# SHI-Labs/SH-GAN

Measured on AMD Instinct MI355X. Metric: generator images/sec, higher is better.
Workload: dtype f32

## Files before the change

### sh-gan_amd/csrc/conv_wino_poly.hip

```cpp
#include "wino_common.h"
#include <stdlib.h>
#include <type_traits>

__device__ __attribute__((aligned(16))) float shg_poly_zeros[64];

struct PolySub {
    const float* wu;
    int nby, nbx;
    int tiles_x, tiles_y;
    int n_ttiles;
};
struct PolyParams {
    const float* x;
    float* y;
    const float* in_scale;
    int NB, I, O, OP, H, W;
    int n_otiles, nchunk;
    PolySub a, b;
    const float* wt;
    int IPK, n_strip_tiles;
    int PH2, PP;
    const float* bias;
    const float* residual;
    int act;
    float alpha, gain, clamp;
    int cps;
    long part_stride;
};

namespace poly {
constexpr int KC = 8, BO = 64, BT = 64;
constexpr int V_SZ = 16 * KC * BT;
constexpr int NT = 1024;
constexpr int NXF = KC;

enum { UA = 0, UB = 1, DA = 2, DB = 3 };

template <int SCHEME, int TY, int TX, int NBX>
struct Geo {
    static constexpr bool A = SCHEME == UA || SCHEME == DA;
    static_assert(NBX > 0 || TY * TX == BT, "64 blocks per tile");
    static_assert(NBX == 0 || A, "flat tiling is for the 3x3 blocks of schemes UA / DA");
    static constexpr int BS = A ? 3 : 2;
    static constexpr int RMAX = NBX ? (NBX - 1 + BT + NBX - 1) / NBX : TY;
    static constexpr int PH = A ? 3 * RMAX + 1 : 2 * TY + 1;
    static constexpr int PW = SCHEME == UA ? ((3 * (NBX ? NBX : TX) + 1 + 3 + 3) / 4) * 4
                            : SCHEME == DA ? (NBX ? ((3 * NBX + 1 + 3) / 4) * 4 : ((3 * TX + 1 + 3 + 3) / 4) * 4)
                            : 2 * TX + 4;
    static constexpr int DB_W0 = 2 * TX, DB_W1 = 2 * TX + 4, DB_W2 = 2 * TX;
    static constexpr int DB_N0 = (2 * TY + 1) * DB_W0, DB_N1 = 2 * TY * DB_W1, DB_N2 = 2 * TY * DB_W2;
    static constexpr int RP = SCHEME == DB ? DB_N0 + DB_N1 + DB_N2 : PH * PW;
    static constexpr int PW4 = PW / 4, PATCH4 = RP / 4, R_SZ = KC * RP;
    static constexpr int NPIECE = (PATCH4 + 63) / 64;
};
}

template <int SCHEME, int TY, int TX, int NBX>
__device__ __forceinline__ void poly_body(const PolyParams& p, const PolySub& q, const int bid, float* __restrict__ Vl,
                                          float* __restrict__ Rl) {
    using namespace poly;
    using G = Geo<SCHEME, TY, TX, NBX>;
    constexpr int PW = G::PW, PW4 = G::PW4, PATCH4 = G::PATCH4, RP = G::RP, R_SZ = G::R_SZ, BS = G::BS, NPIECE = G::NPIECE;
    constexpr bool FLAT = NBX > 0;
    constexpr bool DOWN = SCHEME == DA || SCHEME == DB;
    const int c0 = DOWN ? 0 : blockIdx.y * p.cps, nch = DOWN ? p.nchunk : min(p.cps, p.nchunk - c0), iend = min(p.I, (c0 + nch) * poly::KC);

    const int tid = threadIdx.x;
    const int lane = tid & 63, wave = __builtin_amdgcn_readfirstlane(tid >> 6);
    const int l31 = lane & 31, half = lane >> 5;

    const int nwork = q.n_ttiles * p.n_otiles;
    const int work = shg_xcd_remap(bid, nwork);
    const int otile = work / q.n_ttiles;
    const int ttile = work - otile * q.n_ttiles;
    const int txb = ttile % q.tiles_x;
    const int tyb = (ttile / q.tiles_x) % q.tiles_y;
    const int n = ttile / (q.tiles_x * q.tiles_y);
    const int id0 = txb * BT;
    const int by0 = FLAT ? id0 / (NBX ? NBX : 1) : tyb * TY, bx0 = FLAT ? 0 : txb * TX;
    const int o0 = otile * BO;
    const int HW = DOWN ? p.PH2 * p.PP : p.H * p.W;
    const int wy0 = DOWN ? BS * by0 : BS * by0 - 1;
    const int wx0 = SCHEME == UA ? ((3 * bx0 - 1) & ~3) : SCHEME == DA ? ((3 * bx0) & ~3) : SCHEME == UB ? 2 * bx0 - 4 : 2 * bx0;
    const int coff = (DOWN ? BS * bx0 : BS * bx0 - 1) - wx0;

    const bool xformer = wave < NXF;
    constexpr int NLD = 16 - NXF;
    constexpr int CPL = (KC + NLD - 1) / NLD;
    int roff[NPIECE];
#pragma unroll
    for (int j = 0; j < NPIECE; ++j) {
        const int e = j * 64 + lane;
        if constexpr (SCHEME == DB) {
            constexpr int N0 = G::DB_N0 / 4, N1 = G::DB_N1 / 4, W0 = G::DB_W0 / 4, W1 = G::DB_W1 / 4, W2 = G::DB_W2 / 4;
            const int pl = e < N0 ? 1 : (e < N0 + N1 ? 2 : 3);
            const int r4 = e < N0 ? e : (e < N0 + N1 ? e - N0 : e - N0 - N1);
            const int w4 = pl == 1 ? W0 : (pl == 2 ? W1 : W2);
            const int py = r4 / w4, p4 = r4 - py * w4;
            const int iy = wy0 + py, ix = wx0 + 4 * p4;
            const bool ok = e < PATCH4 && iy < p.PH2 && ix + 3 < p.PP;
            roff[j] = ok ? (pl * p.NB + n) * p.I * HW + iy * p.PP + ix : -1;
        } else {
            const int py = e / PW4, p4 = e - py * PW4;
            const int iy = wy0 + py, ix = wx0 + 4 * p4;
            if constexpr (SCHEME == DA) {
                const bool ok = e < PATCH4 && iy < p.PH2 && ix + 3 < p.PP;
                roff[j] = ok ? n * p.I * HW + iy * p.PP + ix : -1;
            } else {
                const bool ok = e < PATCH4 && iy >= 0 && iy < p.H && ix >= 0 && ix + 3 < p.W;
                roff[j] = ok ? n * p.I * HW + iy * p.W + ix : -1;
            }
        }
    }
    const bool ract_last = lane < PATCH4 - 64 * (NPIECE - 1);
    auto dma_raw = [&](int c, int buf) __attribute__((always_inline)) {
#pragma unroll
        for (int q = 0; q < CPL; ++q) {
            const int k = (wave - NXF) * CPL + q;
            if (k >= KC) continue;
            const int ch = (c0 + c) * KC + k;
            const bool chok = ch < iend;
#pragma unroll
            for (int j = 0; j < NPIECE; ++j) {
                const float* src = (chok && roff[j] >= 0) ? p.x + ((long)roff[j] + (long)ch * HW) : shg_poly_zeros;
                if (j < NPIECE - 1 || ract_last)
                    __builtin_amdgcn_global_load_lds((const __attribute__((address_space(1))) void*)src,
                                                     (__attribute__((address_space(3))) void*)(Rl + buf * R_SZ + k * RP + j * 256), 16, 0, 0);
            }
        }
    };

    constexpr int NU = KC / 4;
    const size_t ustride = (size_t)16 * 64 * KC / 4;
    const f32x4* ubase = reinterpret_cast<const f32x4*>(q.wu + (((size_t)otile * p.nchunk * 16 + wave) * 64 + lane) * KC) + (size_t)c0 * ustride;
    f32x4 ua[NU], ub[NU];
    auto load_u = [&](f32x4 (&dst)[NU], int c) __attribute__((always_inline)) {
#pragma unroll
        for (int j = 0; j < NU; ++j) dst[j] = ubase[(size_t)c * ustride + j];
    };

    const int tty = FLAT ? (id0 + lane) / (NBX ? NBX : 1) - by0 : lane / TX;
    const int ttx = FLAT ? (id0 + lane) % (NBX ? NBX : 1) : lane % TX;
    const float* rbase = Rl + wave * RP + (SCHEME == DB ? 0 : (BS * tty) * PW + BS * ttx + coff);
    float* vbase = Vl + wave * BT + lane;
    float scv[2];
#pragma unroll
    for (int v = 0; v < 2; ++v) {
        const int ch = (v * 64 + lane) * KC + wave;
        scv[v] = (p.in_scale && xformer && ch < p.I) ? p.in_scale[(long)n * p.I + ch] : 1.f;
    }
    auto transform = [&](int c, int buf) __attribute__((always_inline)) {
        const int ca = c0 + c;
        const float sc = __builtin_bit_cast(float, __builtin_amdgcn_readlane(__builtin_bit_cast(int, ca < 64 ? scv[0] : scv[1]), ca & 63));
        const float* rb = rbase + buf * R_SZ;
        float* vb = vbase + buf * V_SZ;
        if constexpr (SCHEME == DB) {
            const float* we = rb + (2 * tty) * G::DB_W0 + 2 * ttx;
#pragma unroll
            for (int cc = 0; cc < 2; ++cc) {
                const float d0 = we[cc] * sc, d1 = we[G::DB_W0 + cc] * sc, d2 = we[2 * G::DB_W0 + cc] * sc;
                vb[(0 * 2 + cc) * KC * BT] = d0 - d1;
                vb[(1 * 2 + cc) * KC * BT] = d1;
                vb[(2 * 2 + cc) * KC * BT] = d2 - d1;
            }
            const float* wo = rb + G::DB_N0 + (2 * tty) * G::DB_W1 + 2 * ttx;
#pragma unroll
            for (int r = 0; r < 2; ++r) {
                const float e0 = wo[r * G::DB_W1] * sc, e1 = wo[r * G::DB_W1 + 1] * sc, e2 = wo[r * G::DB_W1 + 2] * sc;
                vb[(6 + r * 3 + 0) * KC * BT] = e0 - e1;
                vb[(6 + r * 3 + 1) * KC * BT] = e1;
                vb[(6 + r * 3 + 2) * KC * BT] = e2 - e1;
            }
            const float* wq = rb + G::DB_N0 + G::DB_N1 + (2 * tty) * G::DB_W2 + 2 * ttx;
#pragma unroll
            for (int r = 0; r < 2; ++r)
#pragma unroll
                for (int cc = 0; cc < 2; ++cc) vb[(12 + r * 2 + cc) * KC * BT] = wq[r * G::DB_W2 + cc] * sc;
        } else if constexpr (G::A) {
            float f[4][4];
#pragma unroll
            for (int r = 0; r < 4; ++r) {
                const float d0 = rb[r * PW] * sc, d1 = rb[r * PW + 1] * sc, d2 = rb[r * PW + 2] * sc, d3 = rb[r * PW + 3] * sc;
                f[r][0] = d0 - d2; f[r][1] = d1 + d2; f[r][2] = d2 - d1; f[r][3] = d1 - d3;
                if (r == 1) __builtin_amdgcn_sched_barrier(0);
            }
#pragma unroll
            for (int j = 0; j < 4; ++j) {
                vb[(0 * 4 + j) * KC * BT] = f[0][j] - f[2][j];
                vb[(1 * 4 + j) * KC * BT] = f[1][j] + f[2][j];
                vb[(2 * 4 + j) * KC * BT] = f[2][j] - f[1][j];
                vb[(3 * 4 + j) * KC * BT] = f[1][j] - f[3][j];
            }
        } else {
            float d[3][3];
#pragma unroll
            for (int r = 0; r < 3; ++r)
#pragma unroll
                for (int cc = 0; cc < 3; ++cc) d[r][cc] = rb[r * PW + cc] * sc;
#pragma unroll
            for (int cc = 1; cc < 3; ++cc) {
                vb[(0 * 2 + cc - 1) * KC * BT] = d[0][cc] - d[1][cc];
                vb[(1 * 2 + cc - 1) * KC * BT] = d[1][cc];
                vb[(2 * 2 + cc - 1) * KC * BT] = d[2][cc] - d[1][cc];
            }
#pragma unroll
            for (int r = 1; r < 3; ++r) {
                vb[(6 + (r - 1) * 3 + 0) * KC * BT] = d[r][0] - d[r][1];
                vb[(6 + (r - 1) * 3 + 1) * KC * BT] = d[r][1];
                vb[(6 + (r - 1) * 3 + 2) * KC * BT] = d[r][2] - d[r][1];
            }
#pragma unroll
            for (int r = 1; r < 3; ++r)
#pragma unroll
                for (int cc = 1; cc < 3; ++cc) vb[(12 + (r - 1) * 2 + cc - 1) * KC * BT] = d[r][cc];
        }
    };

    f32x16 acc[2][2];
#pragma unroll
    for (int ob = 0; ob < 2; ++ob)
#pragma unroll
        for (int tb = 0; tb < 2; ++tb)
#pragma unroll
            for (int r = 0; r < 16; ++r) acc[ob][tb][r] = 0.f;
    const float* bbase = Vl + (wave * KC + half) * BT + l31;

    load_u(ua, 0);
    if (!xformer) {
        dma_raw(0, 0);
        if (nch > 1) dma_raw(1, 1);
    }
    asm volatile("s_waitcnt vmcnt(0)" ::: "memory");
    __syncthreads();
    if (xformer) transform(0, 0);
    __syncthreads();

    float b[2][2], apend[2];
    auto mma = [&](float a0, float a1, int buf) __attribute__((always_inline)) {
#pragma unroll
        for (int tb = 0; tb < 2; ++tb) acc[0][tb] = __builtin_amdgcn_mfma_f32_32x32x2f32(a0, b[buf][tb], acc[0][tb], 0, 0, 0);
#pragma unroll
        for (int tb = 0; tb < 2; ++tb) acc[1][tb] = __builtin_amdgcn_mfma_f32_32x32x2f32(a1, b[buf][tb], acc[1][tb], 0, 0, 0);
    };
    auto chunk = [&](auto par, int c) __attribute__((always_inline)) {
        constexpr int PAR = decltype(par)::value;
        f32x4 (&ucur)[NU] = PAR ? ub : ua;
        f32x4 (&unxt)[NU] = PAR ? ua : ub;
        const bool more = c + 1 < nch;
        const float* bb = bbase + PAR * V_SZ;
        auto fetch = [&](int ks, int buf) __attribute__((always_inline)) {
#pragma unroll
            for (int tb = 0; tb < 2; ++tb) b[buf][tb] = bb[(ks * 2) * BT + tb * 32];
        };
        fetch(0, 0);
        __builtin_amdgcn_sched_barrier(0);
        if (c > 0) mma(apend[0], apend[1], 1);
        __builtin_amdgcn_sched_barrier(0);
        if (more) load_u(unxt, c + 1);
        if (!xformer) {
            if (c + 2 < nch) dma_raw(c + 2, PAR);
        } else if (more) {
            transform(c + 1, PAR ^ 1);
        }
        __builtin_amdgcn_sched_barrier(0);
#pragma unroll
        for (int ks = 0; ks < KC / 2 - 1; ++ks) {
            fetch(ks + 1, (ks + 1) & 1);
            __builtin_amdgcn_sched_barrier(0);
            mma(ucur[(ks * 2) / 4][(ks * 2) % 4], ucur[(ks * 2 + 1) / 4][(ks * 2 + 1) % 4], ks & 1);
        }
        apend[0] = ucur[(KC - 2) / 4][(KC - 2) % 4];
        apend[1] = ucur[(KC - 1) / 4][(KC - 1) % 4];
        asm volatile("s_waitcnt lgkmcnt(0)" ::: "memory");
        __syncthreads();
    };
    for (int c = 0; c < nch; c += 2) {
        chunk(std::integral_constant<int, 0>{}, c);
        if (c + 1 < nch) chunk(std::integral_constant<int, 1>{}, c + 1);
    }
    mma(apend[0], apend[1], 1);

    float* Mx = Vl;
    const int PWg = DOWN ? p.W : p.W + 1;
    const long plane = DOWN ? (long)p.H * p.W : (long)(p.H + 1) * PWg;
    const int o_l = tid >> 5, t_l = tid & 31;
    f32x2 pre_part[SCHEME == DB ? 4 : 1][2], pre_res[SCHEME == DB ? 4 : 1][2];
    float pre_bias[2] = {0.f, 0.f};
    if constexpr (SCHEME == DB) {
#pragma unroll
        for (int pass = 0; pass < 4; ++pass) {
            const int ob = pass >> 1, t = (pass & 1) * 32 + t_l;
            const int by = by0 + t / TX, bx = bx0 + t % TX;
            const int o = min(o0 + ob * 32 + o_l, p.O - 1);
            if ((pass & 1) == 0) pre_bias[ob] = p.bias ? p.bias[o] : 0.f;
#pragma unroll
            for (int j = 0; j < 2; ++j) {
                pre_part[pass][j] = f32x2{0.f, 0.f};
                pre_res[pass][j] = f32x2{0.f, 0.f};
                if (by < q.nby && bx < q.nbx && 2 * by + j < p.H) {
                    const long off = ((long)n * p.O + o) * plane + (long)(2 * by + j) * PWg + 2 * bx;
                    pre_part[pass][j] = *reinterpret_cast<const f32x2*>(p.y + off);
                    if (p.residual) pre_res[pass][j] = *reinterpret_cast<const f32x2*>(p.residual + off);
                }
            }
        }
    }
#pragma unroll
    for (int pass = 0; pass < 4; ++pass) {
        const int ob = pass >> 1, tb = pass & 1;
#pragma unroll
        for (int r = 0; r < 16; ++r) {
            const int row = (r & 3) + 8 * (r >> 2) + 4 * half;
            Mx[(wave * 32 + row) * 32 + l31] = acc[ob][tb][r];
        }
        __syncthreads();
        float m[16];
#pragma unroll
        for (int xi = 0; xi < 16; ++xi) m[xi] = Mx[(xi * 32 + o_l) * 32 + t_l];
        const int t = tb * 32 + t_l;
        const int by = FLAT ? (id0 + t) / (NBX ? NBX : 1) : by0 + t / TX, bx = FLAT ? (id0 + t) % (NBX ? NBX : 1) : bx0 + t % TX;
        const int o = o0 + ob * 32 + o_l;
        if (o < p.O && by < q.nby && bx < q.nbx) {
            float* yb = p.y + (DOWN ? 0 : blockIdx.y * p.part_stride) + ((long)n * p.O + o) * plane;
            const long pstride = (long)p.NB * p.O * plane;
            if constexpr (G::A) {
                float t3[3][4];
#pragma unroll
                for (int cc = 0; cc < 4; ++cc) {
                    t3[0][cc] = m[0 * 4 + cc] + m[1 * 4 + cc] + m[2 * 4 + cc];
                    t3[1][cc] = m[1 * 4 + cc] - m[2 * 4 + cc];
                    t3[2][cc] = m[1 * 4 + cc] + m[2 * 4 + cc] - m[3 * 4 + cc];
                }
                constexpr int EXT = DOWN ? 0 : 1;
#pragma unroll
                for (int i = 0; i < 3; ++i) {
                    const int u = 3 * by + i;
                    if (u >= p.H + EXT) continue;
                    const float y0 = t3[i][0] + t3[i][1] + t3[i][2], y1 = t3[i][1] - t3[i][2], y2 = t3[i][1] + t3[i][2] - t3[i][3];
                    float* yr = yb + (long)u * PWg + 3 * bx;
                    yr[0] = y0;
                    if (3 * bx + 1 < p.W + EXT) yr[1] = y1;
                    if (3 * bx + 2 < p.W + EXT) yr[2] = y2;
                }
            } else if constexpr (SCHEME == DB) {
                const int p0 = 2 * by, q0 = 2 * bx;
                const float bs = pre_bias[ob];
#pragma unroll
                for (int j = 0; j < 2; ++j) {
                    if (p0 + j >= p.H) continue;
                    float* yr = yb + (long)(p0 + j) * PWg + q0;
                    const f32x2 part = pre_part[pass][j];
                    const f32x2 rs = pre_res[pass][j];
                    f32x2 out;
#pragma unroll
                    for (int cc = 0; cc < 2; ++cc) {
                        float v = part[cc] + m[j * 2 + cc] + m[(j + 1) * 2 + cc]
                                + m[6 + j * 3 + cc] + m[6 + j * 3 + cc + 1]
                                + m[12 + j * 2 + cc] + bs;
                        v = p.act ? shg_lrelu_agc(v, p.alpha, p.gain, p.clamp) : v * p.gain;
                        out[cc] = v + rs[cc];
                    }
                    *reinterpret_cast<f32x2*>(yr) = out;
                }
            } else {
                const int u0 = 2 * by, v0 = 2 * bx;
                float* yeo = yb + pstride + (long)u0 * PWg + v0;
                float* yoe = yb + 2 * pstride + (long)u0 * PWg + v0;
                float* yoo = yb + 3 * pstride + (long)u0 * PWg + v0;
#pragma unroll
                for (int cc = 0; cc < 2; ++cc) {
                    yeo[cc] = m[0 * 2 + cc] + m[1 * 2 + cc];
                    yeo[PWg + cc] = m[1 * 2 + cc] + m[2 * 2 + cc];
                }
#pragma unroll
                for (int r = 0; r < 2; ++r) {
                    yoe[r * PWg] = m[6 + r * 3] + m[6 + r * 3 + 1];
                    yoe[r * PWg + 1] = m[6 + r * 3 + 1] + m[6 + r * 3 + 2];
                    yoo[r * PWg] = m[12 + r * 2];
                    yoo[r * PWg + 1] = m[12 + r * 2 + 1];
                }
            }
        }
        if (pass < 3) __syncthreads();
    }
}

__device__ __forceinline__ void poly_strip_body(const PolyParams& p, const int tile, const int wave, float* __restrict__ redbuf) {
    float (*red)[16][64] = reinterpret_cast<float (*)[16][64]>(redbuf);
    const float* wt = p.wt;
    const int IPK = p.IPK;
    const int lane = threadIdx.x & 63;
    const int l31 = lane & 31, half = lane >> 5;
    const int nseg_r = (p.W + 31) / 32, nseg_c = (p.H + 31) / 32;
    const int no32 = p.OP / 32;
    const bool live = tile < p.n_strip_tiles;
    int seg = tile % (nseg_r + nseg_c);
    const int ot32 = (tile / (nseg_r + nseg_c)) % no32;
    const int n = live ? tile / ((nseg_r + nseg_c) * no32) : 0;
    const bool col = seg >= nseg_r;
    if (col) seg -= nseg_r;
    const int len = col ? p.H : p.W;
    const int pos = seg * 32 + l31;
    const int tap = col ? 1 * 3 + 2 : 2 * 3 + 1;
    const int HW = p.H * p.W;
    const bool pok = live && pos < len;
    const float* xb = p.x + (long)n * p.I * HW + (pok ? (col ? pos * p.W + p.W - 1 : (p.H - 1) * p.W + pos) : 0);
    const float* wb = wt + ((long)(ot32 >> 1) * IPK + tap) * 64 + (ot32 & 1) * 32 + l31;
    const float* sb = p.in_scale ? p.in_scale + (long)n * p.I : nullptr;
    const int i_lo = blockIdx.y * p.cps * poly::KC, i_hi = min(p.I, i_lo + p.cps * poly::KC);
    const int kper = ((i_hi - i_lo + 7) / 8) * 2;
    const int kbeg = i_lo + wave * kper, kend = min(i_hi, kbeg + kper);
    f32x16 acc;
#pragma unroll
    for (int r = 0; r < 16; ++r) acc[r] = 0.f;
    for (int i0 = kbeg; i0 < kend; i0 += 32) {
        float a[16], bv[16];
#pragma unroll
        for (int k = 0; k < 16; ++k) {
            const int ic = i0 + 2 * k + half;
            const int i = min(ic, p.I - 1);
            a[k] = wb[(long)i * 9 * 64];
            bv[k] = xb[(long)i * HW];
            if (sb) bv[k] *= sb[i];
            if (ic >= kend) a[k] = 0.f;
            if (ic >= kend || !pok) bv[k] = 0.f;
        }
#pragma unroll
        for (int k = 0; k < 16; ++k) acc = __builtin_amdgcn_mfma_f32_32x32x2f32(a[k], bv[k], acc, 0, 0, 0);
    }
#pragma unroll
    for (int r = 0; r < 16; ++r) red[wave][r][lane] = acc[r];
    __syncthreads();
    if (!pok) return;
    const int PWg = p.W + 1;
    const long plane = (long)(p.H + 1) * PWg;
    const long pix = col ? (long)pos * PWg + p.W : (long)p.H * PWg + pos;
    float* yb = p.y + blockIdx.y * p.part_stride + (long)(col ? 2 : 1) * p.NB * p.O * plane + (long)n * p.O * plane + pix;
#pragma unroll
    for (int rr = 0; rr < 4; ++rr) {
        const int r = wave * 4 + rr;
        const float v = red[0][r][lane] + red[1][r][lane] + red[2][r][lane] + red[3][r][lane];
        const int o = ot32 * 32 + (r & 3) + 8 * (r >> 2) + 4 * half;
        if (o < p.O) yb[(long)o * plane] = v;
    }
}

template <int ATY, int ATX, int ANBX, int BTY, int BTX>
__global__ __launch_bounds__(1024) void conv_poly_up_kernel(const PolyParams p) {
    using namespace poly;
    using GA = Geo<UA, ATY, ATX, ANBX>;
    using GB = Geo<UB, BTY, BTX, 0>;
    constexpr int R_MAX = GA::R_SZ > GB::R_SZ ? GA::R_SZ : GB::R_SZ;
    __shared__ __attribute__((aligned(16))) float Vl[2 * V_SZ];
    __shared__ __attribute__((aligned(16))) float Rl[2 * R_MAX];
    const int nA = p.a.n_ttiles * p.n_otiles, nB = p.b.n_ttiles * p.n_otiles;
    if ((int)blockIdx.x < nA) poly_body<UA, ATY, ATX, ANBX>(p, p.a, blockIdx.x, Vl, Rl);
    else if ((int)blockIdx.x < nA + nB) poly_body<UB, BTY, BTX, 0>(p, p.b, blockIdx.x - nA, Vl, Rl);
    else {
        const int wave = threadIdx.x >> 6;
        poly_strip_body(p, (blockIdx.x - nA - nB) * 4 + (wave >> 2), wave & 3, Vl + (wave >> 2) * 4 * 16 * 64);
    }
}

template <int SCHEME, int TY, int TX, int NBX>
__global__ __launch_bounds__(1024) void conv_poly_down_kernel(const PolyParams p) {
    using namespace poly;
    using G = Geo<SCHEME, TY, TX, NBX>;
    __shared__ __attribute__((aligned(16))) float Vl[2 * V_SZ];
    __shared__ __attribute__((aligned(16))) float Rl[2 * G::R_SZ];
    poly_body<SCHEME, TY, TX, NBX>(p, SCHEME == DA ? p.a : p.b, blockIdx.x, Vl, Rl);
}

__global__ __launch_bounds__(256) void poly_weight_kernel(const float* w, const float* scale, float* wu, int O, int I, int OP,
                                                          int nchunk, int flip, int scheme) {
    constexpr int KC = poly::KC;
    const long e = (long)blockIdx.x * 256 + threadIdx.x;
    const long total = (long)OP * nchunk * KC;
    if (e >= total) return;
    const int o = (int)(e % OP);
    const int i = (int)(e / OP);
    float g[3][3];
#pragma unroll
    for (int t = 0; t < 9; ++t) {
        const int tt = flip ? 8 - t : t;
        g[t / 3][t % 3] = (o < O && i < I) ? w[((long)o * I + i) * 9 + tt] * scale[o] : 0.f;
    }
    float u[16];
    if (scheme == poly::UA) {
        const float q00 = g[2][2], q01 = g[2][0], q10 = g[0][2], q11 = g[0][0];
        float gq[4][2];
        gq[0][0] = q00; gq[0][1] = q01;
        gq[1][0] = 0.5f * (q00 + q10); gq[1][1] = 0.5f * (q01 + q11);
        gq[2][0] = 0.5f * (q00 - q10); gq[2][1] = 0.5f * (q01 - q11);
        gq[3][0] = q10; gq[3][1] = q11;
#pragma unroll
        for (int r = 0; r < 4; ++r) {
            u[r * 4 + 0] = gq[r][0];
            u[r * 4 + 1] = 0.5f * (gq[r][0] + gq[r][1]);
            u[r * 4 + 2] = 0.5f * (gq[r][0] - gq[r][1]);
            u[r * 4 + 3] = gq[r][1];
        }
    } else if (scheme == poly::UB) {
        const float g0 = g[0][1], g1 = g[2][1];
        const float h0 = g[1][0], h1 = g[1][2];
#pragma unroll
        for (int cc = 0; cc < 2; ++cc) { u[0 * 2 + cc] = g1; u[1 * 2 + cc] = g0 + g1; u[2 * 2 + cc] = g0; }
#pragma unroll
        for (int r = 0; r < 2; ++r) { u[6 + r * 3 + 0] = h1; u[6 + r * 3 + 1] = h0 + h1; u[6 + r * 3 + 2] = h0; }
#pragma unroll
        for (int k = 0; k < 4; ++k) u[12 + k] = g[1][1];
    } else if (scheme == poly::DA) {
        const float q00 = g[0][0], q01 = g[0][2], q10 = g[2][0], q11 = g[2][2];
        float gq[4][2];
        gq[0][0] = q00; gq[0][1] = q01;
        gq[1][0] = 0.5f * (q00 + q10); gq[1][1] = 0.5f * (q01 + q11);
        gq[2][0] = 0.5f * (q00 - q10); gq[2][1] = 0.5f * (q01 - q11);
        gq[3][0] = q10; gq[3][1] = q11;
#pragma unroll
        for (int r = 0; r < 4; ++r) {
            u[r * 4 + 0] = gq[r][0];
            u[r * 4 + 1] = 0.5f * (gq[r][0] + gq[r][1]);
            u[r * 4 + 2] = 0.5f * (gq[r][0] - gq[r][1]);
            u[r * 4 + 3] = gq[r][1];
        }
    } else {
        const float g0 = g[0][1], g1 = g[2][1];
        const float h0 = g[1][0], h1 = g[1][2];
#pragma unroll
        for (int cc = 0; cc < 2; ++cc) { u[0 * 2 + cc] = g0; u[1 * 2 + cc] = g0 + g1; u[2 * 2 + cc] = g1; }
#pragma unroll
        for (int r = 0; r < 2; ++r) { u[6 + r * 3 + 0] = h0; u[6 + r * 3 + 1] = h0 + h1; u[6 + r * 3 + 2] = h1; }
#pragma unroll
        for (int k = 0; k < 4; ++k) u[12 + k] = g[1][1];
    }
    const int k = i % KC, chunk = i / KC;
    const int ln = (k & 1) * 32 + (o & 31), slot = (k >> 1) * 2 + ((o & 63) >> 5);
    float* dst = wu + ((((long)(o >> 6) * nchunk + chunk) * 16) * 64 + ln) * KC + slot;
#pragma unroll
    for (int xi = 0; xi < 16; ++xi) dst[(long)xi * 64 * KC] = u[xi];
}

extern "C" int shg_conv_weight_prep_up_poly_f32(const float* w, const float* wscale, float* wu_a, float* wu_b, int O, int I, int OP,
                                                int flip, void* stream) {
    SHG_CHECK_ARG(w && wscale && wu_a && wu_b, "weight_prep_up_poly: null pointer");
    SHG_CHECK_ARG(O >= 1 && I >= 1 && OP % 64 == 0 && OP >= O, "weight_prep_up_poly: bad shape");
    const int nchunk = shg_cdiv(I, poly::KC);
    const long total = (long)OP * nchunk * poly::KC;
    hipLaunchKernelGGL(poly_weight_kernel, dim3(shg_cdiv(total, 256)), dim3(256), 0, (hipStream_t)stream, w, wscale, wu_a, O, I, OP,
                       nchunk, flip, (int)poly::UA);
    SHG_CHECK_LAUNCH();
    hipLaunchKernelGGL(poly_weight_kernel, dim3(shg_cdiv(total, 256)), dim3(256), 0, (hipStream_t)stream, w, wscale, wu_b, O, I, OP,
                       nchunk, flip, (int)poly::UB);
    SHG_CHECK_LAUNCH();
    return SHG_OK;
}

extern "C" int shg_conv2d_up_poly_supported(int NB, int I, int O, int H, int W) {
    return (H >= 16 && W >= 16 && H % 2 == 0 && W % 4 == 0 && I <= 128 * poly::KC && NB >= 1 && O >= 1) ? 1 : 0;
}

static int up_poly_plan(PolyParams& p, int NB, int I, int OP, int H, int W) {
    p.n_otiles = OP / 64; p.nchunk = shg_cdiv(I, poly::KC);
    const bool bwide = W >= 32;
    p.b.nby = H / 2; p.b.nbx = W / 2;
    p.b.tiles_x = shg_cdiv(p.b.nbx, bwide ? 16 : 8); p.b.tiles_y = shg_cdiv(p.b.nby, bwide ? 4 : 8);
    p.b.n_ttiles = p.b.tiles_x * p.b.tiles_y * NB;
    p.a.nby = shg_cdiv(H + 1, 3); p.a.nbx = shg_cdiv(W + 1, 3);
    const bool flat = bwide && (p.a.nbx == 11 || p.a.nbx == 22 || p.a.nbx == 43);
    const long w88 = (long)shg_cdiv(p.a.nbx, 8) * shg_cdiv(p.a.nby, 8), w416 = (long)shg_cdiv(p.a.nbx, 16) * shg_cdiv(p.a.nby, 4);
    const bool wide = bwide && w416 < w88;
    if (flat) { p.a.tiles_x = shg_cdiv(p.a.nby * p.a.nbx, 64); p.a.tiles_y = 1; }
    else { p.a.tiles_x = shg_cdiv(p.a.nbx, wide ? 16 : 8); p.a.tiles_y = shg_cdiv(p.a.nby, wide ? 4 : 8); }
    p.a.n_ttiles = p.a.tiles_x * p.a.tiles_y * NB;
    p.IPK = (I + 31) / 32 * 32 * 9;
    p.n_strip_tiles = (shg_cdiv(W, 32) + shg_cdiv(H, 32)) * (OP / 32) * NB;
    if (!bwide) return 0;
    if (flat) return p.a.nbx == 11 ? 1 : (p.a.nbx == 22 ? 2 : 3);
    return wide ? 4 : 5;
}

extern "C" size_t shg_conv2d_up_poly_workspace_bytes(int NB, int I, int O, int OP, int H, int W) {
    if (!shg_conv2d_up_poly_supported(NB, I, O, H, W) || OP < 64) return 0;
    PolyParams p{};
    up_poly_plan(p, NB, I, OP, H, W);
    return shg_wino_split_bytes((long)(p.a.n_ttiles + p.b.n_ttiles) * p.n_otiles, p.nchunk, (size_t)4 * NB * O * (H + 1) * (W + 1) * sizeof(float));
}

extern "C" int shg_conv2d_up_poly_ws_f32(const float* x, const float* wt, const float* wu_a, const float* wu_b, float* y, int NB, int I,
                                         int O, int OP, int H, int W, const float* in_scale, void* workspace, size_t ws_bytes, void* stream) {
    SHG_CHECK_ARG(x && wt && wu_a && wu_b && y, "conv2d_up_poly: null pointer");
    SHG_CHECK_ARG(shg_conv2d_up_poly_supported(NB, I, O, H, W), "conv2d_up_poly: unsupported geometry (use shg_conv2d_f32 mode 2)");
    SHG_CHECK_ARG(OP % 64 == 0 && OP >= O, "conv2d_up_poly: OP must be a multiple of 64 and >= O");
    SHG_CHECK_ARG((long)NB * I * H * W < 2147483647L && 4L * NB * O * (H + 1) * (W + 1) < 2147483647L, "conv2d_up_poly: tensor too large");
    SHG_CHECK_ARG((reinterpret_cast<uintptr_t>(x) & 15) == 0, "conv2d_up_poly: x must be 16-byte aligned");
    hipStream_t s = (hipStream_t)stream;
    PolyParams p{};
    p.x = x; p.y = y; p.in_scale = in_scale;
    p.NB = NB; p.I = I; p.O = O; p.OP = OP; p.H = H; p.W = W;
    p.a.wu = wu_a; p.b.wu = wu_b; p.wt = wt;
    const int variant = up_poly_plan(p, NB, I, OP, H, W);
    const int ks = shg_wino_split((long)(p.a.n_ttiles + p.b.n_ttiles) * p.n_otiles, p.nchunk, (size_t)4 * NB * O * (H + 1) * (W + 1) * sizeof(float),
                                  workspace, ws_bytes, shg_addr(workspace) | shg_addr(y), &p.y, &p.cps, &p.part_stride);
    const dim3 grid((p.a.n_ttiles + p.b.n_ttiles) * p.n_otiles + shg_cdiv(p.n_strip_tiles, 4), ks);
    if (variant == 0) hipLaunchKernelGGL((conv_poly_up_kernel<8, 8, 0, 8, 8>), grid, dim3(poly::NT), 0, s, p);
    else if (variant == 1) hipLaunchKernelGGL((conv_poly_up_kernel<1, 64, 11, 4, 16>), grid, dim3(poly::NT), 0, s, p);
    else if (variant == 2) hipLaunchKernelGGL((conv_poly_up_kernel<1, 64, 22, 4, 16>), grid, dim3(poly::NT), 0, s, p);
    else if (variant == 3) hipLaunchKernelGGL((conv_poly_up_kernel<1, 64, 43, 4, 16>), grid, dim3(poly::NT), 0, s, p);
    else if (variant == 4) hipLaunchKernelGGL((conv_poly_up_kernel<4, 16, 0, 4, 16>), grid, dim3(poly::NT), 0, s, p);
    else hipLaunchKernelGGL((conv_poly_up_kernel<8, 8, 0, 4, 16>), grid, dim3(poly::NT), 0, s, p);
    SHG_CHECK_LAUNCH();
    if (ks > 1) {
        shg_launch_wino_split_reduce((const float*)workspace, y, ks, 4 * NB, O, H + 1, W + 1, nullptr, nullptr, nullptr, 0, 0.f, 0, 0.f, 1.f, -1.f, nullptr, s);
        SHG_CHECK_LAUNCH();
    }
    return SHG_OK;
}

extern "C" int shg_conv2d_up_poly_f32(const float* x, const float* wt, const float* wu_a, const float* wu_b, float* y, int NB, int I,
                                      int O, int OP, int H, int W, const float* in_scale, void* stream) {
    return shg_conv2d_up_poly_ws_f32(x, wt, wu_a, wu_b, y, NB, I, O, OP, H, W, in_scale, nullptr, 0, stream);
}


extern "C" int shg_conv_weight_prep_down_poly_f32(const float* w, const float* wscale, float* wu_a, float* wu_b, int O, int I, int OP,
                                                  int flip, void* stream) {
    SHG_CHECK_ARG(w && wscale && wu_a && wu_b, "weight_prep_down_poly: null pointer");
    SHG_CHECK_ARG(O >= 1 && I >= 1 && OP % 64 == 0 && OP >= O, "weight_prep_down_poly: bad shape");
    const int nchunk = shg_cdiv(I, poly::KC);
    const long total = (long)OP * nchunk * poly::KC;
    hipLaunchKernelGGL(poly_weight_kernel, dim3(shg_cdiv(total, 256)), dim3(256), 0, (hipStream_t)stream, w, wscale, wu_a, O, I, OP,
                       nchunk, flip, (int)poly::DA);
    SHG_CHECK_LAUNCH();
    hipLaunchKernelGGL(poly_weight_kernel, dim3(shg_cdiv(total, 256)), dim3(256), 0, (hipStream_t)stream, w, wscale, wu_b, O, I, OP,
                       nchunk, flip, (int)poly::DB);
    SHG_CHECK_LAUNCH();
    return SHG_OK;
}

extern "C" int shg_conv2d_down_poly_supported(int NB, int I, int O, int OH, int OW) {
    return (OH >= 16 && OW >= 16 && OW % 4 == 0 && OH % 2 == 0 && I <= 128 * poly::KC && NB >= 1 && O >= 1) ? 1 : 0;
}

extern "C" int shg_conv2d_down_poly_f32(const float* xp, const float* wu_a, const float* wu_b, float* y, int NB, int I, int O, int OP,
                                        int OH, int OW, int PP, const float* in_scale, const float* bias, int act, float alpha,
                                        float gain, float clamp, const float* residual, void* stream) {
    SHG_CHECK_ARG(xp && wu_a && wu_b && y, "conv2d_down_poly: null pointer");
    SHG_CHECK_ARG(shg_conv2d_down_poly_supported(NB, I, O, OH, OW), "conv2d_down_poly: unsupported geometry (use shg_conv2d_f32 mode 1)");
    SHG_CHECK_ARG(OP % 64 == 0 && OP >= O, "conv2d_down_poly: OP must be a multiple of 64 and >= O");
    SHG_CHECK_ARG(PP % 4 == 0 && PP >= OW + 1, "conv2d_down_poly: plane pitch must be a multiple of 4 and >= OW + 1");
    SHG_CHECK_ARG(4L * NB * I * (OH + 1) * PP < 2147483647L && (long)NB * O * OH * OW < 2147483647L, "conv2d_down_poly: tensor too large");
    SHG_CHECK_ARG(((reinterpret_cast<uintptr_t>(xp) & 15) | (reinterpret_cast<uintptr_t>(y) & 7) | (reinterpret_cast<uintptr_t>(residual) & 7)) == 0,
                  "conv2d_down_poly: xp must be 16-byte, y / residual 8-byte aligned");
    hipStream_t s = (hipStream_t)stream;
    PolyParams p{};
    p.x = xp; p.y = y; p.in_scale = in_scale; p.bias = bias; p.residual = residual;
    p.NB = NB; p.I = I; p.O = O; p.OP = OP; p.H = OH; p.W = OW; p.PH2 = OH + 1; p.PP = PP;
    p.act = act; p.alpha = alpha; p.gain = gain; p.clamp = clamp;
    p.n_otiles = OP / 64; p.nchunk = shg_cdiv(I, poly::KC);
    p.cps = p.nchunk; p.part_stride = 0;
    p.a.wu = wu_a; p.a.nby = shg_cdiv(OH, 3); p.a.nbx = shg_cdiv(OW, 3);
    const bool flat = p.a.nbx == 11 || p.a.nbx == 22 || p.a.nbx == 43;
    const long w88 = (long)shg_cdiv(p.a.nbx, 8) * shg_cdiv(p.a.nby, 8), w416 = (long)shg_cdiv(p.a.nbx, 16) * shg_cdiv(p.a.nby, 4);
    const bool wide = OW >= 32 && w416 < w88;
    if (flat) { p.a.tiles_x = shg_cdiv(p.a.nby * p.a.nbx, 64); p.a.tiles_y = 1; }
    else { p.a.tiles_x = shg_cdiv(p.a.nbx, wide ? 16 : 8); p.a.tiles_y = shg_cdiv(p.a.nby, wide ? 4 : 8); }
    p.a.n_ttiles = p.a.tiles_x * p.a.tiles_y * NB;
    const dim3 ga(p.a.n_ttiles * p.n_otiles);
    if (flat && p.a.nbx == 11) hipLaunchKernelGGL((conv_poly_down_kernel<poly::DA, 1, 64, 11>), ga, dim3(poly::NT), 0, s, p);
    else if (flat && p.a.nbx == 22) hipLaunchKernelGGL((conv_poly_down_kernel<poly::DA, 1, 64, 22>), ga, dim3(poly::NT), 0, s, p);
    else if (flat) hipLaunchKernelGGL((conv_poly_down_kernel<poly::DA, 1, 64, 43>), ga, dim3(poly::NT), 0, s, p);
    else if (wide) hipLaunchKernelGGL((conv_poly_down_kernel<poly::DA, 4, 16, 0>), ga, dim3(poly::NT), 0, s, p);
    else hipLaunchKernelGGL((conv_poly_down_kernel<poly::DA, 8, 8, 0>), ga, dim3(poly::NT), 0, s, p);
    SHG_CHECK_LAUNCH();
    const bool bwide = OW >= 32, bxwide = OW >= 64;
    p.b.wu = wu_b; p.b.nby = OH / 2; p.b.nbx = OW / 2;
    p.b.tiles_x = shg_cdiv(p.b.nbx, bxwide ? 32 : (bwide ? 16 : 8)); p.b.tiles_y = shg_cdiv(p.b.nby, bxwide ? 2 : (bwide ? 4 : 8));
    p.b.n_ttiles = p.b.tiles_x * p.b.tiles_y * NB;
    const dim3 gb(p.b.n_ttiles * p.n_otiles);
    if (bxwide) hipLaunchKernelGGL((conv_poly_down_kernel<poly::DB, 2, 32, 0>), gb, dim3(poly::NT), 0, s, p);
    else if (bwide) hipLaunchKernelGGL((conv_poly_down_kernel<poly::DB, 4, 16, 0>), gb, dim3(poly::NT), 0, s, p);
    else hipLaunchKernelGGL((conv_poly_down_kernel<poly::DB, 8, 8, 0>), gb, dim3(poly::NT), 0, s, p);
    SHG_CHECK_LAUNCH();
    return SHG_OK;
}
```

Measured before the change: 824.5.

## Specialize winograd main loop on transformer role and tighten LDS DMA issue

Splits the chunk loop into two compile-time variants, one for waves that transform and one for waves that issue raw-input DMA, so the runtime branch leaves the hot loop. Replaces the global_load_lds builtin with inline asm that sets M0 from a scalar (readfirstlane) LDS address. Transform outputs now go to registers first and are stored to LDS together at the end. An explicit vmcnt wait is added before the end-of-chunk barrier. The goal is less branching and better instruction scheduling, at the cost of code size and the fragility of hand-written inline asm and waitcnt encodings.

```diff
diff --git a/sh-gan_amd/csrc/conv_wino_poly.hip b/sh-gan_amd/csrc/conv_wino_poly.hip
--- a/sh-gan_amd/csrc/conv_wino_poly.hip
+++ b/sh-gan_amd/csrc/conv_wino_poly.hip
@@ -123,9 +123,10 @@
 #pragma unroll
             for (int j = 0; j < NPIECE; ++j) {
                 const float* src = (chok && roff[j] >= 0) ? p.x + ((long)roff[j] + (long)ch * HW) : shg_poly_zeros;
+                const unsigned lds = __builtin_amdgcn_readfirstlane(
+                    (unsigned)(size_t)(__attribute__((address_space(3))) void*)(Rl + buf * R_SZ + k * RP + j * 256));
                 if (j < NPIECE - 1 || ract_last)
-                    __builtin_amdgcn_global_load_lds((const __attribute__((address_space(1))) void*)src,
-                                                     (__attribute__((address_space(3))) void*)(Rl + buf * R_SZ + k * RP + j * 256), 16, 0, 0);
+                    asm volatile("s_mov_b32 m0, %0\n\ts_nop 0\n\tglobal_load_lds_dwordx4 %1, off" ::"s"(lds), "v"(src) : "m0", "memory");
             }
         }
     };
@@ -150,32 +151,32 @@
         scv[v] = (p.in_scale && xformer && ch < p.I) ? p.in_scale[(long)n * p.I + ch] : 1.f;
     }
     auto transform = [&](int c, int buf) __attribute__((always_inline)) {
+        float tv[16];
         const int ca = c0 + c;
         const float sc = __builtin_bit_cast(float, __builtin_amdgcn_readlane(__builtin_bit_cast(int, ca < 64 ? scv[0] : scv[1]), ca & 63));
         const float* rb = rbase + buf * R_SZ;
-        float* vb = vbase + buf * V_SZ;
         if constexpr (SCHEME == DB) {
             const float* we = rb + (2 * tty) * G::DB_W0 + 2 * ttx;
 #pragma unroll
             for (int cc = 0; cc < 2; ++cc) {
                 const float d0 = we[cc] * sc, d1 = we[G::DB_W0 + cc] * sc, d2 = we[2 * G::DB_W0 + cc] * sc;
-                vb[(0 * 2 + cc) * KC * BT] = d0 - d1;
-                vb[(1 * 2 + cc) * KC * BT] = d1;
-                vb[(2 * 2 + cc) * KC * BT] = d2 - d1;
+                tv[0 * 2 + cc] = d0 - d1;
+                tv[1 * 2 + cc] = d1;
+                tv[2 * 2 + cc] = d2 - d1;
             }
             const float* wo = rb + G::DB_N0 + (2 * tty) * G::DB_W1 + 2 * ttx;
 #pragma unroll
             for (int r = 0; r < 2; ++r) {
                 const float e0 = wo[r * G::DB_W1] * sc, e1 = wo[r * G::DB_W1 + 1] * sc, e2 = wo[r * G::DB_W1 + 2] * sc;
-                vb[(6 + r * 3 + 0) * KC * BT] = e0 - e1;
-                vb[(6 + r * 3 + 1) * KC * BT] = e1;
-                vb[(6 + r * 3 + 2) * KC * BT] = e2 - e1;
+                tv[6 + r * 3 + 0] = e0 - e1;
+                tv[6 + r * 3 + 1] = e1;
+                tv[6 + r * 3 + 2] = e2 - e1;
             }
             const float* wq = rb + G::DB_N0 + G::DB_N1 + (2 * tty) * G::DB_W2 + 2 * ttx;
 #pragma unroll
             for (int r = 0; r < 2; ++r)
 #pragma unroll
-                for (int cc = 0; cc < 2; ++cc) vb[(12 + r * 2 + cc) * KC * BT] = wq[r * G::DB_W2 + cc] * sc;
+                for (int cc = 0; cc < 2; ++cc) tv[12 + r * 2 + cc] = wq[r * G::DB_W2 + cc] * sc;
         } else if constexpr (G::A) {
             float f[4][4];
 #pragma unroll
@@ -186,10 +187,10 @@
             }
 #pragma unroll
             for (int j = 0; j < 4; ++j) {
-                vb[(0 * 4 + j) * KC * BT] = f[0][j] - f[2][j];
-                vb[(1 * 4 + j) * KC * BT] = f[1][j] + f[2][j];
-                vb[(2 * 4 + j) * KC * BT] = f[2][j] - f[1][j];
-                vb[(3 * 4 + j) * KC * BT] = f[1][j] - f[3][j];
+                tv[0 * 4 + j] = f[0][j] - f[2][j];
+                tv[1 * 4 + j] = f[1][j] + f[2][j];
+                tv[2 * 4 + j] = f[2][j] - f[1][j];
+                tv[3 * 4 + j] = f[1][j] - f[3][j];
             }
         } else {
             float d[3][3];
@@ -199,21 +200,24 @@
                 for (int cc = 0; cc < 3; ++cc) d[r][cc] = rb[r * PW + cc] * sc;
 #pragma unroll
             for (int cc = 1; cc < 3; ++cc) {
-                vb[(0 * 2 + cc - 1) * KC * BT] = d[0][cc] - d[1][cc];
-                vb[(1 * 2 + cc - 1) * KC * BT] = d[1][cc];
-                vb[(2 * 2 + cc - 1) * KC * BT] = d[2][cc] - d[1][cc];
+                tv[0 * 2 + cc - 1] = d[0][cc] - d[1][cc];
+                tv[1 * 2 + cc - 1] = d[1][cc];
+                tv[2 * 2 + cc - 1] = d[2][cc] - d[1][cc];
             }
 #pragma unroll
             for (int r = 1; r < 3; ++r) {
-                vb[(6 + (r - 1) * 3 + 0) * KC * BT] = d[r][0] - d[r][1];
-                vb[(6 + (r - 1) * 3 + 1) * KC * BT] = d[r][1];
-                vb[(6 + (r - 1) * 3 + 2) * KC * BT] = d[r][2] - d[r][1];
+                tv[6 + (r - 1) * 3 + 0] = d[r][0] - d[r][1];
+                tv[6 + (r - 1) * 3 + 1] = d[r][1];
+                tv[6 + (r - 1) * 3 + 2] = d[r][2] - d[r][1];
             }
 #pragma unroll
             for (int r = 1; r < 3; ++r)
 #pragma unroll
-                for (int cc = 1; cc < 3; ++cc) vb[(12 + (r - 1) * 2 + cc - 1) * KC * BT] = d[r][cc];
-        }
+                for (int cc = 1; cc < 3; ++cc) tv[12 + (r - 1) * 2 + cc - 1] = d[r][cc];
+        }
+        float* vb = vbase + buf * V_SZ;
+#pragma unroll
+        for (int xi = 0; xi < 16; ++xi) vb[xi * KC * BT] = tv[xi];
     };
 
     f32x16 acc[2][2];
@@ -242,8 +246,9 @@
 #pragma unroll
         for (int tb = 0; tb < 2; ++tb) acc[1][tb] = __builtin_amdgcn_mfma_f32_32x32x2f32(a1, b[buf][tb], acc[1][tb], 0, 0, 0);
     };
-    auto chunk = [&](auto par, int c) __attribute__((always_inline)) {
+    auto chunk = [&](auto par, auto xf_c, int c) __attribute__((always_inline)) {
         constexpr int PAR = decltype(par)::value;
+        constexpr bool XF = decltype(xf_c)::value;
         f32x4 (&ucur)[NU] = PAR ? ub : ua;
         f32x4 (&unxt)[NU] = PAR ? ua : ub;
         const bool more = c + 1 < nch;
@@ -257,7 +262,7 @@
         if (c > 0) mma(apend[0], apend[1], 1);
         __builtin_amdgcn_sched_barrier(0);
         if (more) load_u(unxt, c + 1);
-        if (!xformer) {
+        if constexpr (!XF) {
             if (c + 2 < nch) dma_raw(c + 2, PAR);
         } else if (more) {
             transform(c + 1, PAR ^ 1);
@@ -271,13 +276,18 @@
         }
         apend[0] = ucur[(KC - 2) / 4][(KC - 2) % 4];
         apend[1] = ucur[(KC - 1) / 4][(KC - 1) % 4];
+        __builtin_amdgcn_s_waitcnt(0x0F70);
         asm volatile("s_waitcnt lgkmcnt(0)" ::: "memory");
         __syncthreads();
     };
-    for (int c = 0; c < nch; c += 2) {
-        chunk(std::integral_constant<int, 0>{}, c);
-        if (c + 1 < nch) chunk(std::integral_constant<int, 1>{}, c + 1);
-    }
+    auto run = [&](auto xf_c) __attribute__((always_inline)) {
+        for (int c = 0; c < nch; c += 2) {
+            chunk(std::integral_constant<int, 0>{}, xf_c, c);
+            if (c + 1 < nch) chunk(std::integral_constant<int, 1>{}, xf_c, c + 1);
+        }
+    };
+    if (xformer) run(std::true_type{});
+    else run(std::false_type{});
     mma(apend[0], apend[1], 1);
 
     float* Mx = Vl;
```

Result: no change. 828.9, median of 6 (+0.5%).
